# PBozmarov/RL-Environment-for-Component-Placement

Measured on AMD Instinct MI355X. Metric: env_steps_per_sec, higher is better.
Workload: dtype u64; 1 GPU; c3: 64x64 grid, 16 components, 48 pins, reward=centroid; envs_per_gpu=4096, queue_depth=2, instances=replay, fresh_instance_every_reset=False, incremental_obs=False, loop=fused, store_policy=sc1 (write-through)

## Files before the change

rl-environment-for-component-placement_amd/csrc/pcb_step.h:

```cpp
static __device__ inline void presample_next(const DevParams &p, Lds &l, int sampled, int genv, u64 seed, u64 next_step, int lane) {
    if (lane >= WAVE) return;
#ifdef PCBENV_NO_PRESAMPLE
    sampled = 0;
#endif
    if (!sampled) { if (lane == 0) l.hdr->pre_action = 0u; return; }
    int o, x, y;
    sample_action(l.vm, p, genv, lane, seed, next_step, &o, &x, &y);
    if (lane == 0) {
        l.hdr->pre_seed = seed; l.hdr->pre_step = next_step; l.hdr->pre_genv = (unsigned)genv;
        l.hdr->pre_action = (unsigned)o | ((unsigned)x << 8) | ((unsigned)y << 16) | 0x80000000u;
    }
}

static __device__ __forceinline__ void draw_action(const DevParams &p, Lds &l, int genv, int lane, u64 seed, u64 step, int *o, int *x, int *y) {
    if (lane < WAVE) {
        sample_action(l.vm, p, genv, lane, seed, step, o, x, y);
        if (NT > WAVE && lane == 0) { l.hdr->pad[0] = (unsigned)*o; l.hdr->pad[1] = (unsigned)*x; l.hdr->flag = (unsigned)*y; }
    }
    if (NT > WAVE) {
        lds_sync();
        *o = (int)l.hdr->pad[0]; *x = (int)l.hdr->pad[1]; *y = (int)l.hdr->flag;
    }
}

#define MODE_ALL 0
#define MODE_DELEGATED 1
#define MODE_REWARD 2
#define MODE_FEATURES 3

template <int KIND, int WW, bool ROUTES, bool TRAJ>
static __device__ __forceinline__ void transition(const DevParams &p, Lds &l, int e, int row, int lane, int o, int x, int y, int mode, int part, unsigned pos) {
    const int H = p.H, W = p.W, plane = H * WW;
    const bool auto_reset = p.flags & PCBENV_FLAG_AUTO_RESET;
    if (mode == MODE_FEATURES) { reset_env<KIND, WW, TRAJ>(p, l, e, row, lane, RESET_FEATURES); return; }
    const bool full = TRAJ && p.num_slots > 1;
    const int cur = l.hdr->cur, ncomp = l.hdr->ncomp, npins = l.hdr->npins;
    bool valid = PCB_ACTION_IN_RANGE(o, x, y, p.O, H, W) && (KIND == PCBENV_SQUARE || cur >= 0);
    if (valid) valid = PCB_LEGAL_BIT(l.vm, (o & 1) * plane, WW, x, y);
    if (mode == MODE_REWARD && !valid) return;
    const bool obs = mode != MODE_REWARD;
    const bool helpers_route = mode == MODE_DELEGATED && valid;

    if (lane == 0 && p.buf.info && mode == MODE_ALL) { p.buf.info[2 * (size_t)row] = nan(""); p.buf.info[2 * (size_t)row + 1] = nan(""); }
    if (NT > WAVE) lds_sync();

    bool done = true;
    if (valid && !(helpers_route && auto_reset)) {
        int ph, pw;
        CompRec cr = CompRec();
        if (KIND == PCBENV_SQUARE) ph = pw = p.component_n;
        else {
            cr = l.comps[cur];
            ph = PCB_PLACED_H(o, cr.h, cr.w);
            pw = PCB_PLACED_W(o, cr.h, cr.w);
        }
        for (int r = x + lane; r < x + ph && r < H; r += NT) {
            PCB_OCCUPY_ROW(l.occ, r * WW, WW, y, pw)
        }
        if (KIND != PCBENV_SQUARE) {
            if (lane == 0) { l.comps[cur].px = (signed char)x; l.comps[cur].py = (signed char)y; l.comps[cur].o = (unsigned char)o; }
            if (KIND == PCBENV_PIN || KIND == PCBENV_SPATIAL) {
                const int ch = cr.h, cw = cr.w;
                for (int q = lane; q < npins; q += NT) {
                    PinRec pr = l.pins[q];
                    if (pr.comp != cur) continue;
                    PCB_PLACE_PIN(pr, o, ch, cw, x, y)
                    l.pins[q] = pr;
                    if (!full && obs) write_pin_num<KIND>(p, row, pr);
                }
            }
            if (lane == 0) {
                const int next = next_component(cur, ncomp);
                if (!full && obs) {
                    if (p.buf.all_components_feature) {
                        double *cf = p.buf.all_components_feature + ((size_t)row * p.C + cur) * p.F;
                        cf[2] = x; cf[3] = y;
                    }
                    if (p.buf.placement_mask) {
                        double *pm = p.buf.placement_mask + (size_t)row * p.C;
                        pm[cur] = KIND == PCBENV_RECT ? 1.0 : 2.0;
                        if (next >= 0 && KIND != PCBENV_RECT) pm[next] = 3.0;
                    }
                }
                l.hdr->cur = (short)next;
            }
        }
        lds_sync();
        STAMP(3);
        if (obs) {
            const bool inc = (p.flags & PCBENV_FLAG_INCREMENTAL_OBS) != 0;
            const int r0 = inc ? x : 0, r1 = inc ? min(x + ph, H) : H;
            const bool skip_emit = auto_reset && KIND != PCBENV_SQUARE && l.hdr->cur < 0;
            const bool slot_features = TRAJ && full && !skip_emit;
            const bool from_cache = slot_features && KIND == PCBENV_SPATIAL && feat_cache_valid(p, l, e);
            const bool late = slot_features && (KIND == PCBENV_SPATIAL ? from_cache : KIND == PCBENV_PIN);
            auto emit_slot_features = [&]() {
                if (from_cache) {
                    STAMP(5);
                    emit_features_full<KIND>(p, l, row, lane, true);
                    STAMP(6);
                    feat_cache_emit(p, l, e, row, lane);
                    STAMP(7);
                } else {
                    if (KIND == PCBENV_SPATIAL) build_pin_tables(p, l, lane);
                    emit_features_full<KIND>(p, l, row, lane);
                    if (KIND == PCBENV_SPATIAL) { emit_component_grid(p, l, row, lane); lds_sync(); }
                }
            };
            if (slot_features && !late) emit_slot_features();
            const bool any = mask_and_emit<KIND, WW>(p, l, row, lane, !skip_emit, r0, r1);
            STAMP(23);
            if (KIND == PCBENV_SPATIAL && !skip_emit) emit_pin_grid<WW>(p, l, row, lane, r0, r1);
            STAMP(4);
            if (late) emit_slot_features();
            done = episode_done<KIND>(l.hdr->cur, any);
        }
    } else if (!valid && TRAJ && full && !auto_reset && obs) {
        if (KIND == PCBENV_SPATIAL) build_pin_tables(p, l, lane);
        emit_features_full<KIND>(p, l, row, lane);
        if (KIND == PCBENV_SPATIAL) { emit_component_grid(p, l, row, lane); lds_sync(); }
        mask_and_emit<KIND, WW>(p, l, row, lane, true, 0, H);
        if (KIND == PCBENV_SPATIAL) emit_pin_grid<WW>(p, l, row, lane, 0, H);
    }
    if (mode != MODE_REWARD) {
        if (lane == 0) p.buf.done[row] = done ? 1 : 0;
        if (KIND == PCBENV_SQUARE || KIND == PCBENV_RECT) { if (lane == 0) p.buf.reward[row] = valid ? 1.0 : 0.0; }
        else if (!done) { if (lane == 0) p.buf.reward[row] = 0.0; }
    }
    if ((KIND == PCBENV_PIN || KIND == PCBENV_SPATIAL) && done && !helpers_route)
        terminal_reward<KIND, ROUTES>(p, l, row, lane, part, mode == MODE_REWARD ? REWARD_PARTS : 1, pos);
    STAMP(9);
    if (done && auto_reset && mode != MODE_REWARD) {
        store_drain_sync();
        reset_env<KIND, WW, TRAJ>(p, l, e, row, lane, mode == MODE_DELEGATED ? RESET_STATE_MASKS : RESET_ALL);
    }
    STAMP(10);
}

#define ROLE_ENV 0
#define ROLE_REWARD 1
#define ROLE_FEATURES 2
template <int KIND, int WW, bool ROUTES, bool TRAJ>
static __device__ __forceinline__ void run_env(const DevParams &p_launch, unsigned char *smem, int e, int lane0, int *actions, int fmt, int sampled,
                                               u64 seed, u64 first_env, u64 step_index, int num_steps, int role, int part, unsigned pos) {
    STAMP_ROWS_BY_ENV(p_launch, role == ROLE_ENV ? e : p_launch.B + (int)pos * (REWARD_PARTS + 1) + part);
    const int H = p.H, W = p.W, HW = H * W;
    STAMP_RT(30);
    STAMP(0);
    load_state(smem, p, e, lane0);
    Lds l = carve(smem, p);
    STAMP(1);
    int mode = MODE_ALL;
    if (KIND != PCBENV_SQUARE && p.term_wgs > 0) {
        const u64 mk = ((u64)l.hdr->term_seq << 32) | l.hdr->term_pos;
        const bool listed = (unsigned)(mk >> 32) == p.seq && (unsigned)mk < (unsigned)p.term_wgs && (role == ROLE_ENV || (unsigned)mk == pos);
        const int cur = l.hdr->cur;
        const bool last = cur >= 0 && cur == l.hdr->ncomp - 1;
        if (listed && last) mode = role == ROLE_ENV ? MODE_DELEGATED : role == ROLE_REWARD ? MODE_REWARD : MODE_FEATURES;
        else if (role != ROLE_ENV) return;
    }
    const int genv = (int)first_env + e;
    const size_t per_step = (size_t)p.B * (fmt == PCBENV_ACTION_TUPLE ? 3 : 1);
    int slot = p.slot;
    for (int t = 0; t < num_steps; t++) {
        int lane = lane0;
        asm volatile("" : "+v"(lane));
        int o = 0, x = 0, y = 0;
        int *act = actions + per_step * (size_t)t;
        if (mode == MODE_FEATURES) {
        } else if (sampled) {
            const unsigned pa = l.hdr->pre_action, pg = l.hdr->pre_genv;
            const u64 ps = l.hdr->pre_seed, pst = l.hdr->pre_step;
            if ((t == 0) & (pa >> 31) & (ps == seed) & (pst == step_index) & (pg == (unsigned)genv)) {
                o = (int)(pa & 0xFFu); x = (int)((pa >> 8) & 0xFFu); y = (int)((pa >> 16) & 0xFFu);
                STAMP(21);
            } else {
                draw_action(p, l, genv, lane, seed, step_index + (u64)t, &o, &x, &y);
            }
            if (lane == 0 && role == ROLE_ENV) {
                if (fmt == PCBENV_ACTION_FLAT) act[e] = PCB_FLATTEN_ACTION(o, x, y, HW, W);
                else { act[3 * e] = o; act[3 * e + 1] = x; act[3 * e + 2] = y; }
            }
        } else if (fmt == PCBENV_ACTION_FLAT) {
            unflatten_action(act[e], p.O, HW, W, &o, &x, &y);
        } else {
            o = act[3 * e]; x = act[3 * e + 1]; y = act[3 * e + 2];
            if (KIND == PCBENV_SQUARE) o = 0;
        }
        STAMP(2);
        const unsigned episode = l.hdr->episode;
        transition<KIND, WW, ROUTES, TRAJ>(p, l, e, TRAJ ? out_row(p, slot, e) : e, lane, o, x, y, mode, part, pos);
        if (t + 1 < num_steps) {
            if (l.hdr->episode != episode) store_drain_sync(); else lds_sync();
            if (++slot == p.num_slots) slot = 0;
        }
    }
    if (mode == MODE_REWARD || mode == MODE_FEATURES) { STAMP(11); STAMP_RT(31); return; }
    presample_next(p, l, sampled && num_steps == 1, genv, seed, step_index + 1, lane0);
    if (KIND != PCBENV_SQUARE && p.term_cap > 0 && lane0 == 0) {
        const int cur = l.hdr->cur;
        u64 mark = 0ull;
        if (cur >= 0 && cur == l.hdr->ncomp - 1) {
            const unsigned ring = (p.seq + 1u) & 3u, cps = (unsigned)p.term_cap / TERM_SHARDS;
            const unsigned shard = ((unsigned)e * 0x9E3779B1u) >> (32 - TERM_SHARD_BITS);
            const unsigned idx = atomicAdd(PCB_COLD(p, term_cnt) + (ring * TERM_SHARDS + shard) * TERM_CNT_STRIDE, 1u);
            if (idx < cps) {
                const unsigned mpos = idx * TERM_SHARDS + shard;
                PCB_COLD(p, term_list)[ring * (unsigned)p.term_cap + mpos] = e;
                mark = ((u64)(p.seq + 1u) << 32) | mpos;
            }
        }
        l.hdr->term_seq = (unsigned)(mark >> 32); l.hdr->term_pos = (unsigned)mark;
    }
    STAMP(20);
    store_state(smem, p, e, lane0);
    STAMP(11);
    STAMP_RT(31);
}
```

rl-environment-for-component-placement_amd/csrc/pcb_team_io.h:

```cpp
static __device__ inline void lds_sync() {
    __builtin_amdgcn_fence(__ATOMIC_RELEASE, "workgroup", "local");
    if (NT > WAVE) __builtin_amdgcn_s_barrier(); else __builtin_amdgcn_wave_barrier();
    __builtin_amdgcn_fence(__ATOMIC_ACQUIRE, "workgroup", "local");
}
static __device__ inline void store_drain_sync() {
    asm volatile("s_waitcnt vmcnt(0)" ::: "memory");
    lds_sync();
}
static __device__ inline bool block_any(bool v, unsigned *flag) {
    if (NT == WAVE) return __any(v);
    if (threadIdx.x == 0) *flag = 0;
    lds_sync();
    if (__any(v) && (threadIdx.x & 63) == 0) *flag = 1;
    lds_sync();
    return *flag != 0;
}

template <int WW, bool STREAM> static __device__ inline void emit_plane_(unsigned char *dst, const u64 *bits, int r0, int r1, int W, int lane) {
    if ((W & 15) == 0 && (((uintptr_t)dst) & 15) == 0) {
        const ObsDst d = obs_dst(dst, (long long)r1 * W);
        const int sh = (W & (W - 1)) == 0 ? __ffs(W) - 1 : -1;
        if (PCB_GEO64_UNIT && __builtin_constant_p(r0) && __builtin_constant_p(r1 * W) && r0 == 0 && (r1 * W / 16) % NT == 0 && r1 * W / 16 / NT <= 8) {
            PCB_UNROLL
            for (int k = 0; k < r1 * W / 16 / NT; k++) {
                const int cell = (lane + k * NT) * 16, r = sh >= 0 ? cell >> sh : cell / W, col = cell - r * W;
                unsigned b = (unsigned)(bits[r * WW + (col >> 6)] >> (col & 63)) & 0xFFFFu;
                STORE16<STREAM>(d, (unsigned)cell, expand16(b));
            }
            return;
        }
        for (int c = r0 * W / 16 + lane; c < r1 * W / 16; c += NT) {
            int cell = c * 16, r = sh >= 0 ? cell >> sh : cell / W, col = cell - r * W;
            unsigned b = (unsigned)(bits[r * WW + (col >> 6)] >> (col & 63)) & 0xFFFFu;
            STORE16<STREAM>(d, (unsigned)cell, expand16(b));
        }
    } else {
        for (int i = r0 * W + lane; i < r1 * W; i += NT) {
            int r = i / W, col = i - r * W;
            dst[i] = (unsigned char)((bits[r * WW + (col >> 6)] >> (col & 63)) & 1ull);
        }
    }
}
template <bool STREAM> static __device__ inline void emit_zero_(unsigned char *dst, long long bytes, int lane) {
    if ((bytes & 15) == 0 && (((uintptr_t)dst) & 15) == 0) {
        const ObsDst d = obs_dst(dst, bytes);
        for (int c = lane; c < (int)(bytes / 16); c += NT) STORE16<STREAM>(d, (unsigned)c * 16u, make_uint4(0, 0, 0, 0));
    } else {
        for (long long i = lane; i < bytes; i += NT) dst[i] = 0;
    }
}
template <int WW, bool STREAM> static __device__ inline void emit_plane2_(unsigned char *dst, unsigned char *dst2, const u64 *bits, int H, int W, int lane) {
    if ((W & 15) == 0 && (((uintptr_t)dst) & 15) == 0 && (((uintptr_t)dst2) & 15) == 0) {
        const ObsDst d = obs_dst(dst, (long long)H * W), d2 = obs_dst(dst2, (long long)H * W);
        const int sh = (W & (W - 1)) == 0 ? __ffs(W) - 1 : -1;
        if (__builtin_constant_p(H * W) && __builtin_constant_p(W) && (H * W / 16) % NT == 0 && H * W / 16 / NT <= 8) {
            PCB_UNROLL
            for (int k = 0; k < H * W / 16 / NT; k++) {
                const int cell = (lane + k * NT) * 16, r = sh >= 0 ? cell >> sh : cell / W, col = cell - r * W;
                unsigned b = (unsigned)(bits[r * WW + (col >> 6)] >> (col & 63)) & 0xFFFFu;
                const uint4 v = expand16(b);
                STORE16<STREAM>(d, (unsigned)cell, v);
                STORE16<STREAM>(d2, (unsigned)cell, v);
            }
            return;
        }
        for (int c = lane; c < H * W / 16; c += NT) {
            int cell = c * 16, r = sh >= 0 ? cell >> sh : cell / W, col = cell - r * W;
            unsigned b = (unsigned)(bits[r * WW + (col >> 6)] >> (col & 63)) & 0xFFFFu;
            const uint4 v = expand16(b);
            STORE16<STREAM>(d, (unsigned)cell, v);
            STORE16<STREAM>(d2, (unsigned)cell, v);
        }
    } else {
        emit_plane_<WW, STREAM>(dst, bits, 0, H, W, lane);
        emit_plane_<WW, STREAM>(dst2, bits, 0, H, W, lane);
    }
}
template <int WW> static __device__ inline void emit_plane(unsigned char *dst, const u64 *bits, int r0, int r1, int W, int lane, bool stream) {
    if (stream) emit_plane_<WW, true>(dst, bits, r0, r1, W, lane); else emit_plane_<WW, false>(dst, bits, r0, r1, W, lane);
}
template <int WW> static __device__ inline void emit_plane2(unsigned char *dst, unsigned char *dst2, const u64 *bits, int H, int W, int lane, bool stream) {
    if (stream) emit_plane2_<WW, true>(dst, dst2, bits, H, W, lane); else emit_plane2_<WW, false>(dst, dst2, bits, H, W, lane);
}
static __device__ inline void emit_zero(unsigned char *dst, long long bytes, int lane, bool stream) {
    if (stream) emit_zero_<true>(dst, bytes, lane); else emit_zero_<false>(dst, bytes, lane);
}

template <int WW>
static __device__ inline bool window_mask(const u64 *occ, u64 *hf, u64 *vm, int H, int W, int ph, int pw, int lane, unsigned *flag) {
    if (pcb_layout::fold_across_lanes(WW, NT, H)) {
        u64 a = lane < H ? hfold<1>(Row<1>::load(occ + lane), pw).a : 0ull;
        int s = 1;
        while (2 * s <= ph) { a |= lane_down(a, s, lane); s *= 2; }
        if (s < ph) a |= lane_down(a, ph - s, lane);
        const u64 v = (lane + ph <= H) ? Row<1>{a}.free_below(W - pw + 1).a : 0ull;
        if (lane < H) vm[lane] = v;
        return __any(v != 0ull);
    }
    for (int r = lane; r < H; r += NT) hfold<WW>(Row<WW>::load(occ + r * WW), pw).store(hf + r * WW);
    lds_sync();
    bool any = false;
    for (int r = lane; r < H; r += NT) {
        Row<WW> v = Row<WW>::zero();
        if (r + ph <= H) {
            Row<WW> acc = Row<WW>::load(hf + r * WW);
            for (int k = 1; k < ph; k++) acc = acc | Row<WW>::load(hf + (r + k) * WW);
            v = acc.free_below(W - pw + 1);
        }
        v.store(vm + r * WW);
        any |= v.any();
    }
    return block_any(any, flag);
}
```

rl-environment-for-component-placement_amd/csrc/pcb_transition.h:

```cpp
#pragma once
#include "pcb_records.h"

#define PCB_FLATTEN_ACTION(o, x, y, HW, W) ((o) * (HW) + (x) * (W) + (y))
PCB_HD inline int flatten_action(int o, int x, int y, int HW, int W) { return PCB_FLATTEN_ACTION(o, x, y, HW, W); }
PCB_HD inline void split_action(int a, int HW, int W, int *o, int *x, int *y) {
    *o = a / HW;
    const int r = a - *o * HW;
    *x = r / W; *y = r - *x * W;
}
PCB_HD inline void unflatten_action(int a, int O, int HW, int W, int *o, int *x, int *y) {
    if (a < 0 || a >= O * HW) { *o = -1; *x = *y = 0; }
    else split_action(a, HW, W, o, x, y);
}

#define PCB_ACTION_IN_RANGE(o, x, y, O, H, W) ((o) >= 0 && (o) < (O) && (x) >= 0 && (x) < (H) && (y) >= 0 && (y) < (W))
PCB_HD inline bool action_in_range(int o, int x, int y, int O, int H, int W) { return PCB_ACTION_IN_RANGE(o, x, y, O, H, W); }
#define PCB_LEGAL_BIT(vm, plane_off, WW, x, y) (((vm)[(plane_off) + (x) * (WW) + ((y) >> 6)] >> ((y) & 63)) & 1ull)
PCB_HD inline bool legal_bit(const u64 *vm, int H, int WW, int o, int x, int y) { return PCB_LEGAL_BIT(vm, (o & 1) * (H * WW), WW, x, y); }

#define PCB_PLACED_H(o, ch, cw) (((o) & 1) ? (cw) : (ch))
#define PCB_PLACED_W(o, ch, cw) (((o) & 1) ? (ch) : (cw))
PCB_HD inline void placed_extent(int ch, int cw, int o, int *ph, int *pw) { *ph = PCB_PLACED_H(o, ch, cw); *pw = PCB_PLACED_W(o, ch, cw); }
#define PCB_IMAX(a, b) ((a) > (b) ? (a) : (b))
#define PCB_IMIN(a, b) ((a) < (b) ? (a) : (b))
#define PCB_OCCUPY_ROW(words, first, WW, y, pw) \
    for (int w_ = 0; w_ < (WW); w_++) { \
        const int lo_ = PCB_IMAX(y, 64 * w_) - 64 * w_, hi_ = PCB_IMIN((y) + (pw), 64 * w_ + 64) - 64 * w_;   \
        if (hi_ > lo_) (words)[(first) + w_] |= ((hi_ - lo_) >= 64 ? ~0ull : ((1ull << (hi_ - lo_)) - 1ull)) << lo_; \
    }
PCB_HD inline void occupy_row(u64 *row_words, int WW, int y, int pw) { PCB_OCCUPY_ROW(row_words, 0, WW, y, pw) }

#define PCB_PLACE_PIN(pr, o, ch, cw, x, y) { \
        const int rx_ = (pr).rel_x, ry_ = (pr).rel_y; \
        if ((o) == 1) { (pr).rel_x = ry_; (pr).rel_y = (ch) - rx_ - 1; } \
        else if ((o) == 2) { (pr).rel_x = (ch) - rx_ - 1; (pr).rel_y = (cw) - ry_ - 1; } \
        else if ((o) == 3) { (pr).rel_x = (cw) - ry_ - 1; (pr).rel_y = rx_; } \
        (pr).abs_x = (signed char)((x) + (pr).rel_x); (pr).abs_y = (signed char)((y) + (pr).rel_y); \
    }
PCB_HD inline PinRec place_pin(PinRec pr, int o, int ch, int cw, int x, int y) { PCB_PLACE_PIN(pr, o, ch, cw, x, y) return pr; }
#define PCB_UNROTATE_REL(o, ch, cw, rx, ry) { \
        const int ax_ = (rx), ay_ = (ry); \
        if ((o) == 1) { (rx) = (ch) - 1 - ay_; (ry) = ax_; } \
        else if ((o) == 2) { (rx) = (ch) - 1 - ax_; (ry) = (cw) - 1 - ay_; } \
        else if ((o) == 3) { (rx) = ay_; (ry) = (cw) - 1 - ax_; } \
    }
PCB_HD inline void unrotate_rel(int o, int ch, int cw, int *rx, int *ry) { PCB_UNROTATE_REL(o, ch, cw, *rx, *ry) }

PCB_HD inline int next_component(int cur, int ncomp) { return cur + 1 < ncomp ? cur + 1 : -1; }
template <int KIND> PCB_HD inline bool episode_done(int cur_after, bool any) { return KIND == PCBENV_SQUARE ? !any : (cur_after < 0 || !any); }
```

Measured before the change: 232.5 million env-steps/s.

## Add register-resident row-per-lane transition path with shuffle-based window folds

Adds a specialized transition path for single-word-wide 64-row grids, one wave per env, and pin kinds. Each lane holds its occupancy row in a register, updates it directly, and computes the legal-placement mask with logarithmic horizontal bit folds plus cross-lane shuffle vertical folds. This replaces the shared-memory row-OR loop and its barriers. For square components the rotated mask plane is copied rather than recomputed. It adds a second code path that has to stay consistent with the general one, and it depends on lane_down shuffles being correct.

```diff
diff --git a/rl-environment-for-component-placement_amd/csrc/pcb_step.h b/rl-environment-for-component-placement_amd/csrc/pcb_step.h
--- a/rl-environment-for-component-placement_amd/csrc/pcb_step.h
+++ b/rl-environment-for-component-placement_amd/csrc/pcb_step.h
@@ -27,6 +27,52 @@
 #define MODE_DELEGATED 1
 #define MODE_REWARD 2
 #define MODE_FEATURES 3
+
+template <int KIND, int WW>
+static __device__ __forceinline__ bool plain_transition_from_rows(const DevParams &p, Lds &l, int row, int lane, int o, int x, int y, int cur, int npins) {
+    static_assert(PCB_GEO64_UNIT && NT == WAVE && WW == 1 && pcb_layout::is_pin_kind(KIND), "one row per lane, pin kinds, the geometry-fixed units");
+    const int H = p.H, W = p.W, HW = H * W, plane = H * WW, next = cur + 1;
+    const u64 old_row = l.occ[lane];
+    const CompRec cr = l.comps[cur], nr = l.comps[next];
+    const int ph = PCB_PLACED_H(o, cr.h, cr.w), pw = PCB_PLACED_W(o, cr.h, cr.w);
+    const u64 mine = PCB_ROW_AFTER_UPDATE1(old_row, lane, x, ph, y, pw);
+    l.occ[lane] = mine;
+    STAMP(3);
+    unsigned char *m = p.buf.action_mask ? p.buf.action_mask + (size_t)row * p.O * HW : 0;
+    if (p.buf.grid) emit_plane<WW>(p.buf.grid + (size_t)row * HW, l.occ, 0, H, W, lane, p.stream_stores);
+    if (lane == 0) { l.comps[cur].px = (signed char)x; l.comps[cur].py = (signed char)y; l.comps[cur].o = (unsigned char)o; }
+    const int ch = cr.h, cw = cr.w;
+    for (int q = lane; q < npins; q += NT) {
+        PinRec pr = l.pins[q];
+        if (pr.comp != cur) continue;
+        PCB_PLACE_PIN(pr, o, ch, cw, x, y)
+        l.pins[q] = pr;
+        write_pin_num<KIND>(p, row, pr);
+    }
+    if (lane == 0) {
+        if (p.buf.all_components_feature) {
+            double *cf = p.buf.all_components_feature + ((size_t)row * p.C + cur) * p.F;
+            cf[2] = x; cf[3] = y;
+        }
+        if (p.buf.placement_mask) {
+            double *pm = p.buf.placement_mask + (size_t)row * p.C;
+            pm[cur] = 2.0; pm[next] = 3.0;
+        }
+        l.hdr->cur = (short)next;
+    }
+    const int h = nr.h, w = nr.w;
+    bool any = window_mask_row(mine, l.vm, H, W, h, w, lane);
+    if (m) emit_plane2<WW>(m, m + 2 * HW, l.vm, H, W, lane, p.stream_stores);
+    if (h == w) l.vm[plane + lane] = l.vm[lane];
+    else any |= window_mask_row(mine, l.vm + plane, H, W, w, h, lane);
+    if (m) emit_plane2<WW>(m + HW, m + 3 * HW, l.vm + plane, H, W, lane, p.stream_stores);
+    emit_marginals<KIND, WW>(p, l, row, lane);
+    STAMP(23);
+    lds_sync();
+    if (KIND == PCBENV_SPATIAL) emit_pin_grid<WW>(p, l, row, lane, 0, H);
+    STAMP(4);
+    return episode_done<KIND>(next, any);
+}
 
 template <int KIND, int WW, bool ROUTES, bool TRAJ>
 static __device__ __forceinline__ void transition(const DevParams &p, Lds &l, int e, int row, int lane, int o, int x, int y, int mode, int part, unsigned pos) {
@@ -45,7 +91,14 @@
     if (NT > WAVE) lds_sync();
 
     bool done = true;
-    if (valid && !(helpers_route && auto_reset)) {
+    constexpr bool ROWS_ARM = PCB_GEO64_UNIT && !TRAJ && NT == WAVE && WW == 1 && pcb_layout::is_pin_kind(KIND);
+    bool rows_arm = false;
+    if constexpr (ROWS_ARM) {
+        rows_arm = valid && mode == MODE_ALL && H == WAVE && next_component(cur, ncomp) >= 0 && !(p.flags & PCBENV_FLAG_INCREMENTAL_OBS);
+        if (rows_arm) done = plain_transition_from_rows<KIND, WW>(p, l, row, lane, o, x, y, cur, npins);
+    }
+    if (rows_arm) {
+    } else if (valid && !(helpers_route && auto_reset)) {
         int ph, pw;
         CompRec cr = CompRec();
         if (KIND == PCBENV_SQUARE) ph = pw = p.component_n;
diff --git a/rl-environment-for-component-placement_amd/csrc/pcb_team_io.h b/rl-environment-for-component-placement_amd/csrc/pcb_team_io.h
--- a/rl-environment-for-component-placement_amd/csrc/pcb_team_io.h
+++ b/rl-environment-for-component-placement_amd/csrc/pcb_team_io.h
@@ -112,3 +112,9 @@
     }
     return block_any(any, flag);
 }
+static __device__ inline bool window_mask_row(u64 row, u64 *vm, int H, int W, int ph, int pw, int lane) {
+    const u64 a = rows_vfold(row1_hfold(row, pw), ph, [lane](u64 v, int s) { return lane_down(v, s, lane); });
+    const u64 v = (lane + ph <= H) ? row1_free_below(a, W - pw + 1) : 0ull;
+    if (lane < H) vm[lane] = v;
+    return __any(v != 0ull);
+}
diff --git a/rl-environment-for-component-placement_amd/csrc/pcb_transition.h b/rl-environment-for-component-placement_amd/csrc/pcb_transition.h
--- a/rl-environment-for-component-placement_amd/csrc/pcb_transition.h
+++ b/rl-environment-for-component-placement_amd/csrc/pcb_transition.h
@@ -29,6 +29,24 @@
         if (hi_ > lo_) (words)[(first) + w_] |= ((hi_ - lo_) >= 64 ? ~0ull : ((1ull << (hi_ - lo_)) - 1ull)) << lo_; \
     }
 PCB_HD inline void occupy_row(u64 *row_words, int WW, int y, int pw) { PCB_OCCUPY_ROW(row_words, 0, WW, y, pw) }
+#define PCB_OCCUPIED_ROW1(row, y, pw) ((row) | (((pw) >= 64 ? ~0ull : ((1ull << (pw)) - 1ull)) << (y)))
+PCB_HD inline u64 occupied_row1(u64 row, int y, int pw) { return PCB_OCCUPIED_ROW1(row, y, pw); }
+#define PCB_ROW_AFTER_UPDATE1(row, r, x, ph, y, pw) (((r) >= (x) && (r) < (x) + (ph)) ? PCB_OCCUPIED_ROW1(row, y, pw) : (row))
+PCB_HD inline u64 row_after_update1(u64 row, int r, int x, int ph, int y, int pw) { return PCB_ROW_AFTER_UPDATE1(row, r, x, ph, y, pw); }
+
+PCB_HD inline u64 row1_hfold(u64 f, int pw) {
+    int s = 1;
+    while (2 * s <= pw) { f |= f >> s; s *= 2; }
+    if (s < pw) f |= f >> (pw - s);
+    return f;
+}
+template <class V, class Down> PCB_HD inline V rows_vfold(V a, int ph, Down down) {
+    int s = 1;
+    while (2 * s <= ph) { a = a | down(a, s); s *= 2; }
+    if (s < ph) a = a | down(a, ph - s);
+    return a;
+}
+PCB_HD inline u64 row1_free_below(u64 a, int n) { return n <= 0 ? 0ull : (~a & (n >= 64 ? ~0ull : ((1ull << n) - 1ull))); }
 
 #define PCB_PLACE_PIN(pr, o, ch, cw, x, y) { \
         const int rx_ = (pr).rel_x, ry_ = (pr).rel_y; \
```

Result: faster. 241.5 million env-steps/s, median of 6 (+3.9%).
